# mattmireles/Mamba-ASR

Measured on AMD Instinct MI355X. Metric: encoder audio-frames/sec (ConMamba-large, L=4000), higher is better.
Workload: dtype bf16; 1 GPU; conmamba_large_ctc: encoder forward, 64 utterances x 4000 frames (1000 scan steps) per GPU, random-init weights; global_batch=64, frames_per_utterance=4000, parallelism=utterance shards x1 (no collective in forward), launch=hipGraph replay, streams=2 (join)

## Files before the change

### include/conmamba_hip.h

```cpp
#ifndef CONMAMBA_HIP_H
#define CONMAMBA_HIP_H

#include <stdint.h>

#ifdef __cplusplus
extern "C" {
#endif

#define CM_ABI_VERSION 12

#define CM_OK            0
#define CM_EINVAL       (-1)
#define CM_EUNSUPPORTED (-2)
#define CM_EALIGN       (-3)

typedef enum { CM_F32 = 0, CM_BF16 = 1, CM_F16 = 2 } cm_dtype;

#define CM_SCAN_CHUNK 64

int         cm_abi_version(void);
const char *cm_last_error(void);
int         cm_scan_num_chunks(int seqlen);
#ifdef CM_ABLATE
int         cm_debug_set(int ablation);
// ... 511 lines not shown
    const float *chan_mask;
    int32_t mask_rows, mask_c;
} cm_layernorm_args;

int64_t cm_layernorm_bwd_workspace_floats(int64_t rows, int32_t dim);
int cm_layernorm_fwd(const cm_layernorm_args *args);
int cm_layernorm_bwd(const cm_layernorm_args *args);

typedef struct cm_ln_pw_glu_args {
    int32_t rows, dim;
    const float *x;
    const void  *y;
    const float *ln_g, *ln_b;
    const void  *w;
    const float *bias;
    float *x_out;
    void  *out;
    float alpha, eps;
    void *stream;
} cm_ln_pw_glu_args;

int cm_ln_pw_glu(const cm_ln_pw_glu_args *args);

typedef struct cm_cnn_block1_args {
    int32_t batch, T, F, C;
    int32_t io_dtype;
    int32_t pad_out;
    const float *feats;
    const float *weight;
    const float *bias;
    const float *ln_g, *ln_b;
    float eps, slope;
    void *out;
    void *stream;
} cm_cnn_block1_args;

int cm_cnn_block1(const cm_cnn_block1_args *args);

typedef struct cm_cnn_block2_args {
    int32_t batch, T_in, F_in, C_in, C_out;
    int32_t pad_;
    const void  *in;
    const void  *weight;
    const float *bias;
    const float *ln_g, *ln_b;
    float eps, slope;
// ... 139 lines not shown
```

### mamba_asr_amd/_native.py

```python
from __future__ import annotations

import ctypes as C
import os

_HERE = os.path.dirname(os.path.abspath(__file__))
LIB_PATH = os.environ.get("CM_LIB_PATH") or os.path.join(_HERE, "lib", "libconmamba_hip.so")

CM_F32, CM_BF16, CM_F16 = 0, 1, 2
CM_SCAN_CHUNK = 64
CM_CTC_PREFIX_TILE_C, CM_CTC_PREFIX_TCHUNK = 64, 512
CM_BEAM_SELECT_MAX_B, CM_BEAM_SELECT_CHUNK = 128, 5120
CM_ATTN_STEP_MAX_T, CM_ATTN_STEP_MAX_H = 4096, 32
CM_XATTN_STEP_MAX_T, CM_XATTN_STEP_MAX_H = 8192, 32
ABI_VERSION = 12

i32, i64, vp, fp = C.c_int32, C.c_int64, C.c_void_p, C.c_void_p


class ScanFwdArgs(C.Structure):
    _fields_ = [
        ("batch", i32), ("dim", i32), ("seqlen", i32), ("dstate", i32),
        ("io_dtype", i32), ("bc_dtype", i32), ("delta_softplus", i32), ("reverse_time", i32),
        ("u", vp), ("delta", vp), ("A", fp), ("B", vp), ("C", vp), ("D", fp), ("z", vp), ("delta_bias", fp),
        ("out", vp), ("out_z", vp), ("x", fp),
# ... 157 lines not shown

class DwconvClArgs(C.Structure):
    _fields_ = [
        ("batch", i32), ("dim", i32), ("seqlen", i32), ("ksize", i32), ("pad_left", i32), ("io_dtype", i32),
        ("x", vp), ("weight", fp), ("bias", fp), ("y", vp), ("dy", vp), ("dx", vp), ("dweight", fp), ("dbias", fp), ("partial", fp),
        ("x_bs", i64), ("x_ts", i64), ("y_bs", i64), ("y_ts", i64), ("dy_bs", i64), ("dy_ts", i64), ("dx_bs", i64), ("dx_ts", i64),
        ("stream", vp), ("overwrite", i32), ("reserved0", i32),
    ]


class LayerNormArgs(C.Structure):
    _fields_ = [
        ("rows", i64), ("dim", i32), ("x_dtype", i32), ("y_dtype", i32), ("eps", C.c_float),
        ("x", vp), ("gamma", fp), ("beta", fp), ("y", vp), ("mean", fp), ("rstd", fp),
        ("dy", vp), ("dx", vp), ("dgamma", fp), ("dbeta", fp), ("workspace", fp), ("stream", vp), ("dres", fp),
        ("act", i32), ("act_slope", C.c_float), ("chan_mask", fp), ("mask_rows", i32), ("mask_c", i32),
    ]


class LnPwGluArgs(C.Structure):
    _fields_ = [
        ("rows", i32), ("dim", i32), ("x", fp), ("y", vp), ("ln_g", fp), ("ln_b", fp), ("w", vp), ("bias", fp),
        ("x_out", fp), ("out", vp), ("alpha", C.c_float), ("eps", C.c_float), ("stream", vp),
    ]


class CnnFrontArgs(C.Structure):
    _fields_ = [
        ("batch", i32), ("T", i32), ("F", i32), ("C1", i32), ("C2", i32), ("pad_", i32),
        ("feats", fp), ("w1", fp), ("b1", fp), ("ln1_g", fp), ("ln1_b", fp), ("w2", vp), ("b2", fp), ("ln2_g", fp), ("ln2_b", fp),
        ("eps1", C.c_float), ("eps2", C.c_float), ("slope", C.c_float), ("pad2_", i32), ("out", vp), ("stream", vp),
    ]


class AddLnArgs(C.Structure):
    _fields_ = [
        ("rows", i64), ("dim", i32), ("y_dtype", i32), ("out_dtype", i32), ("out_act", i32),
        ("x", fp), ("y", vp), ("alpha", C.c_float), ("eps1", C.c_float), ("eps2", C.c_float), ("pad2_", i32),
        ("g1", fp), ("b1", fp), ("g2", fp), ("b2", fp), ("x_out", fp), ("out", vp), ("stream", vp),
    ]


class GluDwconvArgs(C.Structure):
    _fields_ = [
        ("batch", i32), ("seqlen", i32), ("dim", i32), ("ksize", i32), ("io_dtype", i32), ("glu_done", i32),
        ("in_", vp), ("weight", fp), ("bias", fp), ("ln_g", fp), ("ln_b", fp), ("eps", C.c_float), ("variant", i32),
# ... 132 lines not shown
    ("cm_wgrad_bf16", C.c_int, [C.POINTER(WgradArgs)]),
    ("cm_scan_cl_bwd", C.c_int, [C.POINTER(ScanClBwdArgs)]),
    ("cm_conv_cl_fwd", C.c_int, [C.POINTER(ConvClArgs)]),
    ("cm_sum_leading", C.c_int, [vp, vp, i32, i64, i32, i32, vp]),
    ("cm_ctc_workspace_floats", C.c_int64, [i32, i32, i32]),
    ("cm_ctc_loss", C.c_int, [C.POINTER(CtcArgs)]),
    ("cm_ctc_beam_workspace_bytes", C.c_int64, [C.POINTER(CtcBeamArgs)]),
    ("cm_ctc_beam_search", C.c_int, [C.POINTER(CtcBeamArgs)]),
    ("cm_ctc_prefix_score", C.c_int, [C.POINTER(CtcPrefixArgs)]),
    ("cm_ctc_prefix_advance", C.c_int, [C.POINTER(CtcPrefixArgs)]),
    ("cm_beam_select_workspace_bytes", C.c_int64, [i32, i32, i32]),
    ("cm_beam_select", C.c_int, [C.POINTER(BeamSelectArgs)]),
    ("cm_attn_step", C.c_int, [C.POINTER(AttnStepArgs)]),
    ("cm_xattn_step", C.c_int, [C.POINTER(XattnStepArgs)]),
    ("cm_bias_act_dropout_bwd_workspace_floats", C.c_int64, [i64, i32]),
    ("cm_bias_act_dropout_fwd", C.c_int, [C.POINTER(FfnElemArgs)]),
    ("cm_bias_act_dropout_bwd", C.c_int, [C.POINTER(FfnElemArgs)]),
    ("cm_conv_cl_bwd_workspace_floats", C.c_int64, [i32, i32, i32]),
    ("cm_conv_cl_bwd", C.c_int, [C.POINTER(ConvClBwdArgs)]),
    ("cm_conv_xproj", C.c_int, [C.POINTER(ConvXprojArgs)]),
    ("cm_add_layernorm", C.c_int, [C.POINTER(AddLnArgs)]),
    ("cm_glu_dwconv_ln_gelu", C.c_int, [C.POINTER(GluDwconvArgs)]),
    ("cm_ln_pw_glu", C.c_int, [C.POINTER(LnPwGluArgs)]),
    ("cm_causal_conv1d_update", C.c_int, [C.POINTER(ConvUpdateArgs)]),
    ("cm_selective_state_update", C.c_int, [C.POINTER(StateUpdateArgs)]),
    ("cm_mamba_step", C.c_int, [C.POINTER(MambaStepArgs)]),
    ("cm_layernorm_bwd_workspace_floats", C.c_int64, [i64, i32]),
    ("cm_layernorm_fwd", C.c_int, [C.POINTER(LayerNormArgs)]),
    ("cm_layernorm_bwd", C.c_int, [C.POINTER(LayerNormArgs)]),
    ("cm_dwconv_cl_workspace_floats", C.c_int64, [i32, i32, i32]),
    ("cm_dwconv_cl_fwd", C.c_int, [C.POINTER(DwconvClArgs)]),
    ("cm_dwconv_cl_bwd", C.c_int, [C.POINTER(DwconvClArgs)]),
    ("cm_dwconv1d_fwd", C.c_int, [C.POINTER(Dwconv1dArgs)]),
    ("cm_dwconv1d_bwd", C.c_int, [C.POINTER(Dwconv1dArgs)]),
    ("cm_cnn_block1", C.c_int, [C.POINTER(CnnBlock1Args)]),
    ("cm_cnn_block2", C.c_int, [C.POINTER(CnnBlock2Args)]),
    ("cm_cnn_front", C.c_int, [C.POINTER(CnnFrontArgs)]),
    ("cm_gemm_bf16", C.c_int, [C.POINTER(GemmArgs)]),
    ("cm_ffn_fused", C.c_int, [C.POINTER(FfnArgs)]),
    ("cm_ffn_pack_weights", C.c_int, [vp, i32, i32, vp, vp]),
    ("cm_fbank_mel_db", C.c_int, [C.POINTER(FbankArgs)]),
    ("cm_fbank_finish", C.c_int, [C.POINTER(FbankArgs)]),
    ("cm_fbank_wav", C.c_int, [C.POINTER(FbankArgs)]),
    ("cm_spec_drop", C.c_int, [C.POINTER(SpecDropArgs)]),
]

# ... 31 lines not shown
```

### mamba_asr_amd/csrc/ln_pw_glu.hip

```cpp
#include "cm_common.h"


namespace {

typedef __attribute__((ext_vector_type(8))) __bf16 bf16x8;
typedef __attribute__((ext_vector_type(2))) __bf16 bf16x2;
typedef __attribute__((ext_vector_type(4))) float f32x4;
typedef __attribute__((ext_vector_type(2))) float f32x2;

constexpr int D = 256;
constexpr int TOK = 64;
constexpr int XS = 264;

__device__ __forceinline__ void lds_barrier() { asm volatile("s_waitcnt lgkmcnt(0)\n\ts_barrier" ::: "memory"); }
__device__ __forceinline__ uint32_t pack2(float a, float b) {
    return __builtin_bit_cast(uint32_t, __builtin_convertvector(f32x2{a, b}, bf16x2));
}

template <int OCC, int PF>
__global__ __launch_bounds__(256, OCC) void ln_pw_glu_kernel(const cm_ln_pw_glu_args p) {
    __shared__ __attribute__((aligned(16))) uint16_t xn[TOK * XS];
    const int tid = threadIdx.x, lane = tid & 63;
    const int wave = __builtin_amdgcn_readfirstlane(tid >> 6);
    const int l15 = lane & 15, lq = lane >> 4;
    const int t0 = blockIdx.x * TOK, M = p.rows;
    const uint16_t *yv = reinterpret_cast<const uint16_t *>(p.y);

    const __amdgpu_buffer_rsrc_t wr = __builtin_amdgcn_make_buffer_rsrc(const_cast<void *>(p.w), 0, 2 * D * D * 2, 0x00020000);
    const int vl = lane * 16;
    auto wload = [&](int ps, int s, bf16x8(&dst)[2]) {
        const int half = s >> 3, ks = s & 7;
#pragma unroll
        for (int mb = 0; mb < 2; ++mb)
            dst[mb] = __builtin_bit_cast(bf16x8, __builtin_amdgcn_raw_buffer_load_b128(
                                                     wr, vl, (((half * D + wave * 64) / 16 + 2 * ps + mb) * (D / 32) + ks) * 1024, 0));
    };
    bf16x8 wq[PF][2];
#pragma unroll
    for (int s = 0; s < PF; ++s) wload(0, s, wq[s]);

    {
        float4 v[4][4];
#pragma unroll
        for (int rd = 0; rd < 4; ++rd) {
            const int tok = min(t0 + wave * 16 + rd * 4 + lq, M - 1);
#pragma unroll
            for (int i = 0; i < 4; ++i) {
                const int col = (l15 + 16 * i) * 4;
                float4 x4 = *reinterpret_cast<const float4 *>(p.x + (int64_t)tok * D + col);
                if (yv) {
                    const uint2 a = *reinterpret_cast<const uint2 *>(yv + (int64_t)tok * D + col);
                    x4.x = fmaf(p.alpha, cm_bf16_lo(a.x), x4.x);
                    x4.y = fmaf(p.alpha, cm_bf16_hi(a.x), x4.y);
                    x4.z = fmaf(p.alpha, cm_bf16_lo(a.y), x4.z);
                    x4.w = fmaf(p.alpha, cm_bf16_hi(a.y), x4.w);
                }
                v[rd][i] = x4;
            }
        }
#pragma unroll
        for (int rd = 0; rd < 4; ++rd) {
            const int tok = t0 + wave * 16 + rd * 4 + lq;
            if (p.x_out && tok < M) {
#pragma unroll
                for (int i = 0; i < 4; ++i) *reinterpret_cast<float4 *>(p.x_out + (int64_t)tok * D + (l15 + 16 * i) * 4) = v[rd][i];
            }
            float s = 0.f;
#pragma unroll
            for (int i = 0; i < 4; ++i) s += (v[rd][i].x + v[rd][i].y) + (v[rd][i].z + v[rd][i].w);
            const float mean = cm_group_sum<16>(s) * (1.f / D);
            float q = 0.f;
#pragma unroll
            for (int i = 0; i < 4; ++i) {
                v[rd][i].x -= mean; v[rd][i].y -= mean; v[rd][i].z -= mean; v[rd][i].w -= mean;
                q = fmaf(v[rd][i].x, v[rd][i].x, fmaf(v[rd][i].y, v[rd][i].y, fmaf(v[rd][i].z, v[rd][i].z, fmaf(v[rd][i].w, v[rd][i].w, q))));
            }
            const float rstd = rsqrtf(cm_group_sum<16>(q) * (1.f / D) + p.eps);
            uint16_t *dst = xn + (wave * 16 + rd * 4 + lq) * XS;
#pragma unroll
            for (int i = 0; i < 4; ++i) {
                const int col = (l15 + 16 * i) * 4;
                const float4 g = *reinterpret_cast<const float4 *>(p.ln_g + col);
                const float4 b = *reinterpret_cast<const float4 *>(p.ln_b + col);
                uint2 pk;
                pk.x = pack2(fmaf(v[rd][i].x * rstd, g.x, b.x), fmaf(v[rd][i].y * rstd, g.y, b.y));
                pk.y = pack2(fmaf(v[rd][i].z * rstd, g.z, b.z), fmaf(v[rd][i].w * rstd, g.w, b.w));
                *reinterpret_cast<uint2 *>(dst + col) = pk;
            }
        }
    }
    lds_barrier();

    const uint16_t *xfrag = xn + l15 * XS + lq * 8;
    auto read_frags = [&](int ks, bf16x8(&bf)[4]) {
#pragma unroll
        for (int nb = 0; nb < 4; ++nb) bf[nb] = *reinterpret_cast<const bf16x8 *>(xfrag + nb * 16 * XS + ks * 32);
    };
    uint16_t *out = reinterpret_cast<uint16_t *>(p.out);
    uint2 held[2][4];
#pragma unroll
    for (int ps = 0; ps < 2; ++ps) {
        f32x4 acc[2][2][4];
#pragma unroll
        for (int h = 0; h < 2; ++h)
#pragma unroll
            for (int mb = 0; mb < 2; ++mb)
#pragma unroll
                for (int nb = 0; nb < 4; ++nb) acc[h][mb][nb] = f32x4{0.f, 0.f, 0.f, 0.f};
        bf16x8 bfa[4], bfb[4];
        read_frags(0, bfa);
#pragma unroll
        for (int s = 0; s < 16; ++s) {
// ... 32 lines not shown
    lds_barrier();
#pragma unroll
    for (int i = 0; i < TOK * 32 / 256; ++i) {
        const int idx = tid + 256 * i, row = idx >> 5, chunk = idx & 31;
        const uint4 v = *reinterpret_cast<const uint4 *>(xn + row * XS + chunk * 8);
        if (t0 + row < M) *reinterpret_cast<uint4 *>(out + (int64_t)(t0 + row) * D + chunk * 8) = v;
    }
}

}

extern "C" int cm_ln_pw_glu(const cm_ln_pw_glu_args *args) {
    CM_REQUIRE(args != nullptr, CM_EINVAL, "ln_pw_glu: args is NULL");
    const cm_ln_pw_glu_args &a = *args;
    CM_REQUIRE(a.rows > 0 && a.x && a.ln_g && a.ln_b && a.w && a.bias && a.out, CM_EINVAL, "ln_pw_glu: bad sizes or NULL tensor");
    CM_REQUIRE(a.dim == D, CM_EUNSUPPORTED, "ln_pw_glu: d_model must be 256 (got %d)", a.dim);
    CM_REQUIRE(cm_aligned(a.x, 16) && cm_aligned(a.ln_g, 16) && cm_aligned(a.ln_b, 16) && cm_aligned(a.w, 16) && cm_aligned(a.bias, 16) &&
                   cm_aligned(a.out, 16) && (!a.y || cm_aligned(a.y, 8)) && (!a.x_out || cm_aligned(a.x_out, 16)),
               CM_EALIGN, "ln_pw_glu: tensors must be 16-byte aligned (y / out 8)");
    const dim3 grid((a.rows + TOK - 1) / TOK);
    hipStream_t st = reinterpret_cast<hipStream_t>(a.stream);
#ifdef CM_ABLATE
    if (cm_debug_get() == 41) {
        hipLaunchKernelGGL((ln_pw_glu_kernel<3, 4>), grid, dim3(256), 0, st, a);
        return cm_launch_status("cm_ln_pw_glu");
    }
#endif
    hipLaunchKernelGGL((ln_pw_glu_kernel<4, 2>), grid, dim3(256), 0, st, a);
    return cm_launch_status("cm_ln_pw_glu");
}
```

### mamba_asr_amd/fused.py

```python
from __future__ import annotations

import os
from typing import Dict, Optional

import torch
import torch.nn.functional as F

from . import ops, weight_cache


class _LayerCache:

    def __init__(self, layer, dtype):
        self.dtype = dtype
        c = lambda t: t.detach().to(dtype).contiguous()
        f = lambda t: None if t is None else t.detach().float().contiguous()
        ffn = lambda m: dict(ln=(f(m[0].weight), f(m[0].bias), m[0].eps), w1=c(m[1].ffn[0].weight), b1=c(m[1].ffn[0].bias),
                             w2=c(m[1].ffn[3].weight), b2=c(m[1].ffn[3].bias), b1f=f(m[1].ffn[0].bias),
                             b2f=f(m[1].ffn[3].bias))
        self.ffn1, self.ffn2 = ffn(layer.ffn_module1), ffn(layer.ffn_module2)
        if ops.ffn_supported(self.ffn1["w1"].shape[1], self.ffn1["w1"].shape[0], dtype) and self.ffn1["w1"].is_cuda:
            for q in (self.ffn1, self.ffn2):
                q["w1p"], q["w2p"] = ops.PackedWeight(q["w1"], ops.FFN_LAYOUT), ops.PackedWeight(q["w2"], ops.FFN_LAYOUT)
                if ops.SMALL_FFN_ROWS > 0:
# ... 21 lines not shown
            self.dirs.append(dict(conv_w=f(conv.weight).reshape(m.d_inner, -1), conv_b=f(conv.bias), x_proj=c(xp.weight),
                                  dt_proj=c(dtp.weight), dt_proj_f32=c(dtp.weight).float().contiguous(), dt_bias=f(dtp.bias), A=(-torch.exp(A_log.detach().float())).contiguous(),
                                  D=f(getattr(m, "D_b" if sfx else "D"))))
        cm = layer.convolution_module
        self.x_proj_bd = torch.block_diag(m.x_proj.weight.detach().to(dtype), m.x_proj_b.weight.detach().to(dtype))
        R, N = self.dt_rank, self.d_state
        self.rows_mode = (R <= 16 or (R <= 32 and dtype == torch.bfloat16)) and N == 16 and m.d_inner % 8 == 0
        if self.rows_mode:
            pad = ops.rows_dt_pad(R)
            self.row_width = pad + 32
            rows = [ops.xproj_rows(xp.weight, R, pad, dtype) for xp in (m.x_proj, m.x_proj_b)]
            self.x_proj_rows = torch.block_diag(*rows)
            self.wx_packed = None
            if dtype == torch.bfloat16 and m.d_inner % 32 == 0 and m.d_inner <= 2048 and rows[0].is_cuda and m.d_conv == 4:
                self.wx_packed = [ops.PackedWeight(r) for r in rows]
            for d_, dtp in zip(self.dirs, (m.dt_proj, m.dt_proj_b)):
                d_["dt_w16"] = ops.pad_dt_weight(dtp.weight.detach().to(dtype))
        self.cm_ln = (f(cm.layer_norm.weight), f(cm.layer_norm.bias), cm.layer_norm.eps)
        self.pw_w, self.pw_b = c(cm.bottleneck[0].weight.squeeze(-1)), c(cm.bottleneck[0].bias)
        self.pw_bf, self.lin_bf = f(cm.bottleneck[0].bias), f(cm.after_conv[2].bias)
        self.pw_packed = None
        if dtype == torch.bfloat16 and self.pw_w.is_cuda and tuple(self.pw_w.shape) == (512, 256) and self.pw_bf is not None:
            self.pw_packed = ops.PackedWeight(self.pw_w)
        self.in_bias_f = None if m.in_proj.bias is None else f(m.in_proj.bias)
        self.out_bias_f = None if m.out_proj.bias is None else f(m.out_proj.bias)
        self.dw_w, self.dw_b = f(cm.conv.weight), f(cm.conv.bias)
        self.dw_wt = self.dw_w.reshape(self.dw_w.shape[0], -1).t().contiguous()
        self.cm_ln2 = (f(cm.after_conv[0].weight), f(cm.after_conv[0].bias), cm.after_conv[0].eps)
        self.lin_w, self.lin_b = c(cm.after_conv[2].weight), c(cm.after_conv[2].bias)
        self.lin_packed = None
        if USE_DWCONV_LIN and dtype == torch.bfloat16 and self.lin_w.is_cuda and tuple(self.lin_w.shape) == (256, 256) and self.lin_bf is not None:
            self.lin_packed = ops.PackedWeight(self.lin_w)
        self.kernel_size = cm.kernel_size


def _params_key(dtype, *modules):
    return (dtype,) + tuple((p._version, p.data_ptr()) for m in modules for p in m.parameters())


_LAYER = weight_cache.Kind("_cm_fused_cache", graphs_read=False, build=_LayerCache)


def _cache(layer, dtype) -> _LayerCache:
    return _LAYER.lookup(layer, _params_key(dtype, layer), dtype)


# ... 31 lines not shown
    if c.rows_mode and USE_SCAN_ROWS:
        if xdbl is None:
            xdbl = (ucat.view(rows, 2 * E) @ c.x_proj_rows.t()).view(batch, seqlen, 2 * c.row_width)
        RW = c.row_width
        return [dict(u=ucat[:, :, i * E:(i + 1) * E], A=d["A"], D=d["D"], delta_bias=d["dt_bias"], dt_weight=d["dt_w16"],
                     xdbl=xdbl[:, :, RW * i:RW * (i + 1)], out=ycat[:, :, i * E:(i + 1) * E], reverse=bool(i))
                for i, d in enumerate(c.dirs)]
    xdblT = c.x_proj_bd @ ucat.view(rows, 2 * E).t()
    feat = ops.alloc_bc(2 * P, batch, seqlen, ucat.device)
    feat.view(2 * P, rows).copy_(xdblT)
    dirs = []
    for i, d in enumerate(c.dirs):
        f = feat[i * P:(i + 1) * P]
        dd = dict(u=ucat[:, :, i * E:(i + 1) * E], A=d["A"], B=f[R:R + N], C=f[R + N:], D=d["D"],
                  delta_bias=d["dt_bias"], out=ycat[:, :, i * E:(i + 1) * E], reverse=bool(i))
        if R <= 16:
            dd.update(dt_low=f[:R], dt_weight=d["dt_proj_f32"])
        else:
            dd["delta"] = (xdblT[i * P:i * P + R].t() @ d["dt_proj"].t()).view(batch, seqlen, E)
        dirs.append(dd)
    return dirs


def bimamba_fused(c: _LayerCache, h, batch, seqlen, xz=None):
    E, R, N = c.d_inner, c.dt_rank, c.d_state
    rows = batch * seqlen
    if xz is None:
        xz = h @ c.in_proj.t()
        if c.in_bias is not None:
            xz = xz + c.in_bias
    xz3 = xz.view(batch, seqlen, 2 * E)
    ucat = torch.empty((batch, seqlen, 2 * E), dtype=xz.dtype, device=xz.device)
    xdbl = None
    if USE_CONV_XPROJ and USE_SCAN_ROWS and c.rows_mode and c.wx_packed is not None and xz.dtype == torch.bfloat16:
        xdbl = ops.conv_xproj(xz3[:, :, :E], c.dirs[0]["conv_w"], c.dirs[0]["conv_b"], c.dirs[1]["conv_w"], c.dirs[1]["conv_b"],
                              c.wx_packed[0], c.wx_packed[1], out_f=ucat[:, :, :E], out_b=ucat[:, :, E:])
    else:
        ops.conv_cl_fwd(xz3[:, :, :E], c.dirs[0]["conv_w"], c.dirs[0]["conv_b"], c.dirs[1]["conv_w"], c.dirs[1]["conv_b"],
                        True, out_f=ucat[:, :, :E], out_b=ucat[:, :, E:])
    ycat = torch.empty_like(ucat)
    dirs = _scan_dirs(c, ucat, ycat, batch, seqlen, xdbl)
    ops.scan_cl_fwd(dirs, z=xz3[:, :, E:], delta_softplus=True)
    y = ycat.view(rows, 2 * E) @ c.out_cat.t()
    if c.out_bias is not None:
        y = y + c.out_bias
    if c.gamma is not None:
        y = y * c.gamma.to(y.dtype)
    return y


USE_FUSED_FFN = os.environ.get("CM_FUSED_FFN", "1") == "1"


USE_LN_PW_GLU = os.environ.get("CM_LN_PW_GLU", "1") == "1"


def _layer_forward_ffn_fused(c, x, batch, seqlen, dtype, final_ln=None):
    D = x.shape[-1]
    f1, f2 = c.ffn1, c.ffn2
    if 0 < x.shape[0] <= ops.SMALL_FFN_ROWS and "w1s" in f1:
        f1 = dict(f1, w1p=f1["w1s"], w2p=f1["w2s"])
        f2 = dict(f2, w1p=f2["w1s"], w2p=f2["w2s"])
        inp = getattr(c, "in_packed_s", None)
    else:
        inp = c.in_packed
    if c.in_packed is not None:
        _, xz = ops.ffn_fused(x, f1["ln"], f1["w1p"], f1["b1f"], f1["w2p"], f1["b2f"], alpha=0.5, norm2=c.norm1, proj_w=inp)
        y = bimamba_fused(c, None, batch, seqlen, xz=xz)
    else:
        _, h = ops.ffn_fused(x, f1["ln"], f1["w1p"], f1["b1f"], f1["w2p"], f1["b2f"], alpha=0.5, norm2=c.norm1)
        y = bimamba_fused(c, h, batch, seqlen)
    if USE_LN_PW_GLU and c.pw_packed is not None and y.dtype == torch.bfloat16 and y.is_contiguous():
        gl = ops.ln_pw_glu(x, y, 1.0, c.cm_ln, c.pw_packed, c.pw_bf)
        g = ops.glu_dwconv_ln_gelu(gl.view(batch, seqlen, D), c.dw_w, c.dw_b, c.cm_ln2[0], c.cm_ln2[1], c.cm_ln2[2],
                                   weight_t=c.dw_wt, glu_done=True, lin_w=c.lin_packed, lin_b=c.lin_bf)
    else:
        _, h = ops.add_layernorm(x, y, 1.0, x_out=x, norm2=c.cm_ln, out_dtype=dtype)
        pw = torch.addmm(c.pw_b, h, c.pw_w.t()).view(batch, seqlen, 2 * D)
        g = ops.glu_dwconv_ln_gelu(pw, c.dw_w, c.dw_b, c.cm_ln2[0], c.cm_ln2[1], c.cm_ln2[2], weight_t=c.dw_wt,
                                   lin_w=c.lin_packed, lin_b=c.lin_bf)
    y = g if c.lin_packed is not None else torch.addmm(c.lin_b, g.view(-1, D), c.lin_w.t())
    if final_ln is not None:
        _, out = ops.ffn_fused(x, f2["ln"], f2["w1p"], f2["b1f"], f2["w2p"], f2["b2f"], alpha=0.5, addend=y.view(-1, D),
                               norm1=c.norm2, norm2=final_ln, h_dtype=torch.float32)
        return out, None
    ops.ffn_fused(x, f2["ln"], f2["w1p"], f2["b1f"], f2["w2p"], f2["b2f"], alpha=0.5, addend=y.view(-1, D), norm1=c.norm2,
                  want_h=False)
    return x, None


def layer_forward(layer, x, batch, seqlen, dtype, next_ln=None, final_ln=None):
    c = _cache(layer, dtype)
    D = x.shape[-1]
    if USE_FUSED_FFN and ops.ffn_supported(D, c.ffn1["w1"].shape[0], dtype) and c.ffn2["w1"].shape[0] == c.ffn1["w1"].shape[0]:
        return _layer_forward_ffn_fused(c, x, batch, seqlen, dtype, final_ln)
    _, h = ops.add_layernorm(x, None, norm2=c.ffn1["ln"], out_dtype=dtype)
# ... 102 lines not shown
                        ops.ffn_fused(xp, f1["ln"], f1["w1p"], f1["b1f"], f1["w2p"], f1["b2f"], alpha=0.5, norm2=c.norm1,
                                      proj_w=c.in_packed, proj_out=xz[b0:b1].view(-1, 2 * E))
                    else:
                        _, h = ops.ffn_fused(xp, f1["ln"], f1["w1p"], f1["b1f"], f1["w2p"], f1["b2f"], alpha=0.5, norm2=c.norm1)
                        torch.mm(h, c.in_proj.t(), out=xz[b0:b1].view(-1, 2 * E))
                    ops.conv_xproj(xz[b0:b1, :, :E], c.dirs[0]["conv_w"], c.dirs[0]["conv_b"], c.dirs[1]["conv_w"], c.dirs[1]["conv_b"],
                                   c.wx_packed[0], c.wx_packed[1], out_f=ucat[b0:b1, :, :E], out_b=ucat[b0:b1, :, E:], xdbl=xdbl[b0:b1])
            if paired:
                for pi, (b0, b1) in enumerate(parts):
                    with torch.cuda.stream(streams[pi]):
                        if gate is not None:
                            streams[pi].wait_event(gate)
                        ops.scan_cl_fwd(_scan_dirs(c, ucat[b0:b1], ycat[b0:b1], b1 - b0, seqlen, xdbl[b0:b1]), z=xz[b0:b1, :, E:],
                                        delta_softplus=True)
                        gate = torch.cuda.Event()
                        gate.record(streams[pi])
            else:
                join()
                ops.scan_cl_fwd(_scan_dirs(c, ucat, ycat, batch, seqlen, xdbl), z=xz[:, :, E:], delta_softplus=True)
                fork()
            for pi, (b0, b1) in enumerate(parts):
                with torch.cuda.stream(streams[pi]):
                    xp = x[b0 * seqlen:b1 * seqlen]
                    y = ycat[b0:b1].view(-1, 2 * E) @ c.out_cat.t()
                    gl = ops.ln_pw_glu(xp, y, 1.0, c.cm_ln, c.pw_packed, c.pw_bf)
                    g = ops.glu_dwconv_ln_gelu(gl.view(b1 - b0, seqlen, D), c.dw_w, c.dw_b, c.cm_ln2[0], c.cm_ln2[1], c.cm_ln2[2],
                                               weight_t=c.dw_wt, glu_done=True, lin_w=c.lin_packed, lin_b=c.lin_bf)
                    yl = g.view(-1, D) if c.lin_packed is not None else torch.addmm(c.lin_b, g.view(-1, D), c.lin_w.t())
                    if li == n - 1:
                        _, outs[pi] = ops.ffn_fused(xp, f2["ln"], f2["w1p"], f2["b1f"], f2["w2p"], f2["b2f"], alpha=0.5, addend=yl,
                                                    norm1=c.norm2, norm2=fin, h_dtype=torch.float32)
                    else:
                        ops.ffn_fused(xp, f2["ln"], f2["w1p"], f2["b1f"], f2["w2p"], f2["b2f"], alpha=0.5, addend=yl, norm1=c.norm2,
                                      want_h=False)
        join()
        for o in outs[1:]:
            o.record_stream(cur)
        return torch.cat(outs, dim=0).view(batch, seqlen, D)


@torch.no_grad()
def encoder_forward(encoder, src, dtype: Optional[torch.dtype] = None, streams: Optional[int] = None):
    if dtype is None:
        dtype = torch.get_autocast_dtype("cuda") if torch.is_autocast_enabled("cuda") else torch.float32
    ns = min(N_STREAMS, max(1, src.shape[0] // 16)) if streams is None else streams
    if ns > 1 and src.shape[0] >= 2 * 8 and STREAM_MODE in ("join", "pair"):
        out = _encoder_forward_joined(encoder, src, dtype, ns, paired=STREAM_MODE == "pair")
        if out is not None:
# ... 116 lines not shown
```

### mamba_asr_amd/ops.py

```python
from __future__ import annotations

import ctypes as ct
from typing import Optional, Tuple

import math
import os

import torch

from . import _native as N
from . import weight_cache
from .weight_cache import invalidate_caches

_DT = {torch.float32: N.CM_F32, torch.bfloat16: N.CM_BF16, torch.float16: N.CM_F16}


DETERMINISTIC = os.environ.get("CM_DETERMINISTIC", "1") == "1"


LAUNCH_LOG: Optional[list] = None


def _launch(name: str, fn, args, units: int = 0):
    log = LAUNCH_LOG
# ... 1315 lines not shown
class LnActDropFn(torch.autograd.Function):

    @staticmethod
    def forward(ctx, x, weight, bias, eps, slope, chan_mask, out_dtype):
        b, t, f, c = x.shape
        x2 = x.reshape(b * t, f * c)
        y, x2s, stats = layernorm_fwd(x2, weight, bias, eps, out_dtype, leaky_slope=slope, chan_mask=chan_mask, mask_rows=t)
        ctx.save_for_backward(x2s, stats, weight, bias, chan_mask if chan_mask is not None else weight.new_empty(0))
        ctx.cfg = (eps, slope, t, chan_mask is not None, x.shape)
        return y.view(x.shape)

    @staticmethod
    def backward(ctx, dy):
        x2, stats, weight, bias, mask = ctx.saved_tensors
        eps, slope, t, has_mask, shape = ctx.cfg
        if dy.dtype not in (torch.float32, torch.bfloat16):
            dy = dy.float()
        dy = dy if dy.is_contiguous() else dy.contiguous()
        dx, dg, db = layernorm_bwd(dy.view(x2.shape[0], -1), x2, stats, weight, eps, need_dx=ctx.needs_input_grad[0], bias=bias, leaky_slope=slope,
                                   chan_mask=mask if has_mask else None, mask_rows=t)
        return (dx.view(shape) if dx is not None else None), dg.to(weight.dtype), db.to(weight.dtype), None, None, None, None


def ln_pw_glu(x, y, alpha, norm, w, bias, x_out=None):
    _dev_check(x, y, bias)
    rows, d = x.shape
    if x.dtype != torch.float32 or not x.is_contiguous() or d != 256:
        raise RuntimeError("ln_pw_glu: x must be a contiguous fp32 (rows, 256) tensor")
    if y is not None and (y.dtype != torch.bfloat16 or not y.is_contiguous() or y.shape != x.shape):
        raise RuntimeError("ln_pw_glu: y must be a contiguous bf16 (rows, 256) tensor")
    if not isinstance(w, PackedWeight) or w.shape != (512, 256):
        raise RuntimeError("ln_pw_glu: w must be a PackedWeight of shape (512, 256)")
    g_, b_, bs = _f32c(norm[0]), _f32c(norm[1]), _f32c(bias)
    xo = x if x_out is None else x_out
    out = torch.empty((rows, d), dtype=torch.bfloat16, device=x.device)
    a = N.LnPwGluArgs()
    a.rows, a.dim, a.x, a.y, a.ln_g, a.ln_b, a.w, a.bias = rows, d, _ptr(x), _ptr(y), _ptr(g_), _ptr(b_), _ptr(w.data), _ptr(bs)
    a.x_out, a.out, a.alpha, a.eps, a.stream = _ptr(xo), _ptr(out), float(alpha), float(norm[2]), _stream()
    _launch("cm_ln_pw_glu", N.lib().cm_ln_pw_glu, a, units=rows)
    return out


def glu_dwconv_ln_gelu(inp, weight, bias, ln_weight, ln_bias, eps=1e-5, weight_t=None, glu_done=False, lin_w=None, lin_b=None,
                       variant: int = 0):
    _dev_check(inp, weight, bias, ln_weight, ln_bias)
    if not inp.is_contiguous():
        inp = inp.contiguous()
    b, l, d2 = inp.shape
    d = d2 if glu_done else d2 // 2
    w = _f32c(weight).reshape(d, -1)
    bs, g, bt = _f32c(bias), _f32c(ln_weight), _f32c(ln_bias)
    out = torch.empty((b, l, d), dtype=inp.dtype, device=inp.device)
    a = N.GluDwconvArgs()
    a.batch, a.seqlen, a.dim, a.ksize, a.io_dtype, a.glu_done = b, l, d, w.shape[1], _DT[inp.dtype], int(bool(glu_done))
    a.in_, a.weight, a.bias, a.ln_g, a.ln_b, a.eps, a.out = _ptr(inp), _ptr(w), _ptr(bs), _ptr(g), _ptr(bt), float(eps), _ptr(out)
    wt = w.t().contiguous() if weight_t is None else weight_t
    if wt.dtype != torch.float32 or wt.shape != (w.shape[1], d) or not wt.is_contiguous():
        raise RuntimeError("glu_dwconv_ln_gelu: weight_t must be a contiguous fp32 (k, dim) tensor")
# ... 326 lines not shown
```

### mamba_asr_amd/seqpar.py

```python
from __future__ import annotations

from typing import List, Optional, Sequence, Tuple

import torch
import torch.distributed as dist
import torch.nn.functional as F


class DistGroup:

    def __init__(self, group=None):
        self.group = group
        self.rank, self.world = dist.get_rank(group), dist.get_world_size(group)

    def all_gather(self, t: torch.Tensor) -> List[torch.Tensor]:
        out = [torch.empty_like(t) for _ in range(self.world)]
        dist.all_gather(out, t.contiguous(), group=self.group)
        return out


class _ThreadRank:
    def __init__(self, shared, rank, world):
        self._s, self.rank, self.world = shared, rank, world

# ... 174 lines not shown
            xz = (h @ c.in_proj.t()).view(batch, T, 2 * E)
            left, right = exchange_halo(xz[:, :, :E], 3, 3, group, dim=1)
            xext = torch.cat([left, xz[:, :, :E], right], dim=1)
            uext = torch.empty((batch, T + 6, 2 * E), dtype=dtype, device=dev)
            xdbl_ext = ops.conv_xproj(xext, c.dirs[0]["conv_w"], c.dirs[0]["conv_b"], c.dirs[1]["conv_w"], c.dirs[1]["conv_b"],
                                      c.wx_packed[0], c.wx_packed[1], out_f=uext[:, :, :E], out_b=uext[:, :, E:])
            ucat, xdbl = uext[:, 3:3 + T], xdbl_ext[:, 3:3 + T]
            ycat = torch.empty((batch, T, 2 * E), dtype=dtype, device=dev)
            summ = torch.empty((2, 2, batch, E, 16), dtype=torch.float32, device=dev)
            dirs = [dict(u=ucat[:, :, i * E:(i + 1) * E], A=d["A"], D=d["D"], delta_bias=d["dt_bias"], dt_weight=d["dt_w16"],
                         xdbl=xdbl[:, :, 48 * i:48 * (i + 1)], out=ycat[:, :, i * E:(i + 1) * E], reverse=bool(i),
                         decay=summ[i, 0], h_last=summ[i, 1]) for i, d in enumerate(c.dirs)]
            ops.scan_cl_fwd(dirs, z=xz[:, :, E:], delta_softplus=True)
            allsum = group.all_gather(summ)
            redo = []
            for i in range(2):
                H = carry_in([s_[i, 0] for s_ in allsum], [s_[i, 1] for s_ in allsum], group.rank, bool(i))
                if H is not None:
                    dd = {k: v for k, v in dirs[i].items() if k not in ("decay", "h_last")}
                    dd["h0"] = H.contiguous()
                    redo.append(dd)
            if redo:
                ops.scan_cl_fwd(redo, z=xz[:, :, E:], delta_softplus=True)
            y = ycat.view(batch * T, 2 * E) @ c.out_cat.t()
            gl = ops.ln_pw_glu(x, y, 1.0, c.cm_ln, c.pw_packed, c.pw_bf)
            gl3 = gl.view(batch, T, D)
            left, right = exchange_halo(gl3, 15, 15, group, dim=1)
            g = ops.glu_dwconv_ln_gelu(torch.cat([left, gl3, right], dim=1), c.dw_w, c.dw_b, c.cm_ln2[0], c.cm_ln2[1], c.cm_ln2[2],
                                       weight_t=c.dw_wt, glu_done=True)[:, 15:15 + T]
            yl = torch.addmm(c.lin_b, g.reshape(-1, D), c.lin_w.t())
            if li == len(caches) - 1:
                _, out = ops.ffn_fused(x, f2["ln"], f2["w1p"], f2["b1f"], f2["w2p"], f2["b2f"], alpha=0.5, addend=yl, norm1=c.norm2,
                                       norm2=fin, h_dtype=torch.float32)
            else:
                ops.ffn_fused(x, f2["ln"], f2["w1p"], f2["b1f"], f2["w2p"], f2["b2f"], alpha=0.5, addend=yl, norm1=c.norm2, want_h=False)
        return out.view(batch, T, D)


def exchange_bytes_per_layer(batch: int, d_model: int, expand: int = 2, d_state: int = 16, d_conv: int = 4, kernel_size: int = 31,
                             itemsize: int = 4) -> int:
    E = expand * d_model
    scan = 2 * 2 * batch * E * d_state * 4
    halos = 2 * batch * E * (d_conv - 1) * itemsize + batch * d_model * (kernel_size - 1) * itemsize
    return scan + halos
```

Baseline: 20.67 million audio-frames/s.

## Fuse Mamba out-projection GEMM into the LayerNorm/pointwise-GLU kernel

Adds a MIX variant of the ln_pw_glu kernel that computes the bidirectional-Mamba out-projection (ycat @ out_cat^T) in-kernel. The ycat tiles are streamed into LDS with double-buffered buffer_load...lds DMA, and the projection weights are prefetched into registers. The bf16 result lands in the shared token tile and feeds the residual-add/LayerNorm/pointwise-GLU path, so the separate hipBLAS GEMM and its (rows,256) bf16 intermediate round-trip to HBM go away. The trade-off is more per-block work and register pressure in a kernel that keeps occupancy 4, and the GEMM now runs with a 64-token tile and only 256 threads per block.

```diff
diff --git a/include/conmamba_hip.h b/include/conmamba_hip.h
--- a/include/conmamba_hip.h
+++ b/include/conmamba_hip.h
@@ -557,6 +557,23 @@
 
 int cm_ln_pw_glu(const cm_ln_pw_glu_args *args);
 
+typedef struct cm_ln_pw_glu_mix_args {
+    int32_t rows, dim;
+    const float *x;
+    const float *ln_g, *ln_b;
+    const void  *w;
+    const float *bias;
+    float *x_out;
+    void  *out;
+    float alpha, eps;
+    void *stream;
+    const void *ycat;
+    const void *proj_w;
+    int32_t proj_k;
+} cm_ln_pw_glu_mix_args;
+
+int cm_ln_pw_glu_mix(const cm_ln_pw_glu_mix_args *args);
+
 typedef struct cm_cnn_block1_args {
     int32_t batch, T, F, C;
     int32_t io_dtype;
diff --git a/mamba_asr_amd/_native.py b/mamba_asr_amd/_native.py
--- a/mamba_asr_amd/_native.py
+++ b/mamba_asr_amd/_native.py
@@ -203,6 +203,14 @@
     _fields_ = [
         ("rows", i32), ("dim", i32), ("x", fp), ("y", vp), ("ln_g", fp), ("ln_b", fp), ("w", vp), ("bias", fp),
         ("x_out", fp), ("out", vp), ("alpha", C.c_float), ("eps", C.c_float), ("stream", vp),
+    ]
+
+
+class LnPwGluMixArgs(C.Structure):
+    _fields_ = [
+        ("rows", i32), ("dim", i32), ("x", fp), ("ln_g", fp), ("ln_b", fp), ("w", vp), ("bias", fp),
+        ("x_out", fp), ("out", vp), ("alpha", C.c_float), ("eps", C.c_float), ("stream", vp),
+        ("ycat", vp), ("proj_w", vp), ("proj_k", i32),
     ]
 
 
@@ -381,6 +389,7 @@
     ("cm_add_layernorm", C.c_int, [C.POINTER(AddLnArgs)]),
     ("cm_glu_dwconv_ln_gelu", C.c_int, [C.POINTER(GluDwconvArgs)]),
     ("cm_ln_pw_glu", C.c_int, [C.POINTER(LnPwGluArgs)]),
+    ("cm_ln_pw_glu_mix", C.c_int, [C.POINTER(LnPwGluMixArgs)]),
     ("cm_causal_conv1d_update", C.c_int, [C.POINTER(ConvUpdateArgs)]),
     ("cm_selective_state_update", C.c_int, [C.POINTER(StateUpdateArgs)]),
     ("cm_mamba_step", C.c_int, [C.POINTER(MambaStepArgs)]),
diff --git a/mamba_asr_amd/csrc/ln_pw_glu.hip b/mamba_asr_amd/csrc/ln_pw_glu.hip
--- a/mamba_asr_amd/csrc/ln_pw_glu.hip
+++ b/mamba_asr_amd/csrc/ln_pw_glu.hip
@@ -7,6 +7,7 @@
 typedef __attribute__((ext_vector_type(2))) __bf16 bf16x2;
 typedef __attribute__((ext_vector_type(4))) float f32x4;
 typedef __attribute__((ext_vector_type(2))) float f32x2;
+typedef __attribute__((ext_vector_type(4))) unsigned int u32x4;
 
 constexpr int D = 256;
 constexpr int TOK = 64;
@@ -17,8 +18,30 @@
     return __builtin_bit_cast(uint32_t, __builtin_convertvector(f32x2{a, b}, bf16x2));
 }
 
-template <int OCC, int PF>
-__global__ __launch_bounds__(256, OCC) void ln_pw_glu_kernel(const cm_ln_pw_glu_args p) {
+constexpr int CK = 128;
+constexpr int STAGE = TOK * CK * 2;
+static_assert(2 * STAGE <= TOK * XS * 2, "the two ycat stages must fit the token tile they overlay");
+
+struct mix_extra {
+    const void *ycat;
+    const void *proj_w;
+    int32_t proj_k;
+};
+
+__device__ __forceinline__ u32x4 raw_rsrc(const void *base, uint32_t bytes) {
+    const uint64_t a = reinterpret_cast<uint64_t>(base);
+    return u32x4{(uint32_t)a, (uint32_t)(a >> 32) & 0xffffu, bytes, 0x00020000u};
+}
+__device__ __forceinline__ void dma16(const u32x4 rsrc, uint32_t lds_addr, int voff) {
+    uint32_t keep;
+    asm volatile("s_mov_b32 %0, m0\n\ts_mov_b32 m0, %1\n\ts_nop 0\n\tbuffer_load_dwordx4 %2, %3, 0 offen lds\n\ts_mov_b32 m0, %0"
+                 : "=&s"(keep)
+                 : "s"(lds_addr), "v"(voff), "s"(rsrc)
+                 : "memory");
+}
+
+template <int OCC, int PF, bool MIX>
+__global__ __launch_bounds__(256, OCC) void ln_pw_glu_kernel(const cm_ln_pw_glu_args p, const mix_extra mx) {
     __shared__ __attribute__((aligned(16))) uint16_t xn[TOK * XS];
     const int tid = threadIdx.x, lane = tid & 63;
     const int wave = __builtin_amdgcn_readfirstlane(tid >> 6);
@@ -36,8 +59,77 @@
                                                      wr, vl, (((half * D + wave * 64) / 16 + 2 * ps + mb) * (D / 32) + ks) * 1024, 0));
     };
     bf16x8 wq[PF][2];
-#pragma unroll
-    for (int s = 0; s < PF; ++s) wload(0, s, wq[s]);
+    if constexpr (MIX) {
+        static_assert(PF == 2, "the projection phase's ring indexing assumes two steps in flight");
+        const int K = mx.proj_k, kt = K / 32, nch = K / CK, nstep = 2 * kt;
+        const __amdgpu_buffer_rsrc_t pr = __builtin_amdgcn_make_buffer_rsrc(const_cast<void *>(mx.proj_w), 0, D * K * 2, 0x00020000);
+        auto pload = [&](int g, bf16x8(&dst)[2]) {
+            g = min(g, nstep - 1);
+            const int ks = g >> 1, mp = g & 1;
+#pragma unroll
+            for (int mb = 0; mb < 2; ++mb)
+                dst[mb] = __builtin_bit_cast(bf16x8, __builtin_amdgcn_raw_buffer_load_b128(pr, vl, ((wave * 4 + mp * 2 + mb) * kt + ks) * 1024, 0));
+        };
+        const int vrows = min(TOK, M - t0);
+        const u32x4 yr = raw_rsrc(reinterpret_cast<const unsigned char *>(mx.ycat) + (int64_t)t0 * K * 2, (uint32_t)(vrows * K * 2));
+        const uint32_t lds0 = (uint32_t)reinterpret_cast<uintptr_t>(&xn[0]);
+        int go[4];
+#pragma unroll
+        for (int i = 0; i < 4; ++i) {
+            const int row = 4 * (4 * wave + i) + lq;
+            go[i] = row * K * 2 + 16 * (l15 ^ (((row & 3) << 2) | ((row >> 2) & 3)));
+        }
+        auto request = [&](int c) {
+#pragma unroll
+            for (int i = 0; i < 4; ++i) dma16(yr, lds0 + (uint32_t)((c & 1) * STAGE + (4 * wave + i) * 1024), go[i] + c * (CK * 2));
+        };
+        request(0);
+#pragma unroll
+        for (int s = 0; s < PF; ++s) pload(s, wq[s]);
+        f32x4 acc[4][4];
+#pragma unroll
+        for (int mb = 0; mb < 4; ++mb)
+#pragma unroll
+            for (int nb = 0; nb < 4; ++nb) acc[mb][nb] = f32x4{0.f, 0.f, 0.f, 0.f};
+        const unsigned char *xb = reinterpret_cast<const unsigned char *>(xn);
+        const int yrow = l15 * (CK * 2), yswz = ((l15 & 3) << 2) | (l15 >> 2);
+        auto read_y = [&](int st, int kk, bf16x8(&bf)[4]) {
+            const int off = st * STAGE + yrow + 16 * ((kk * 4 + lq) ^ yswz);
+#pragma unroll
+            for (int nb = 0; nb < 4; ++nb) bf[nb] = *reinterpret_cast<const bf16x8 *>(xb + off + nb * 16 * (CK * 2));
+        };
+        for (int c = 0; c < nch; ++c) {
+            asm volatile("s_waitcnt vmcnt(0)" ::: "memory");
+            lds_barrier();
+            if (c + 1 < nch) request(c + 1);
+            const int st = c & 1;
+            bf16x8 bf[4];
+#pragma unroll
+            for (int s = 0; s < 8; ++s) {
+                const int kk = s >> 1, mp = s & 1;
+                if (mp == 0) read_y(st, kk, bf);
+#pragma unroll
+                for (int mb = 0; mb < 2; ++mb)
+#pragma unroll
+                    for (int nb = 0; nb < 4; ++nb)
+                        acc[mp * 2 + mb][nb] = __builtin_amdgcn_mfma_f32_16x16x32_bf16(wq[s % PF][mb], bf[nb], acc[mp * 2 + mb][nb], 0, 0, 0);
+                pload(c * 8 + s + PF, wq[s % PF]);
+                __builtin_amdgcn_sched_barrier(0);
+            }
+        }
+        lds_barrier();
+#pragma unroll
+        for (int mb = 0; mb < 4; ++mb)
+#pragma unroll
+            for (int nb = 0; nb < 4; ++nb)
+                *reinterpret_cast<uint2 *>(xn + (nb * 16 + l15) * XS + wave * 64 + mb * 16 + lq * 4) =
+                    uint2{pack2(acc[mb][nb][0], acc[mb][nb][1]), pack2(acc[mb][nb][2], acc[mb][nb][3])};
+    }
+    if constexpr (MIX) lds_barrier();
+    else {
+#pragma unroll
+        for (int s = 0; s < PF; ++s) wload(0, s, wq[s]);
+    }
 
     {
         float4 v[4][4];
@@ -48,8 +140,9 @@
             for (int i = 0; i < 4; ++i) {
                 const int col = (l15 + 16 * i) * 4;
                 float4 x4 = *reinterpret_cast<const float4 *>(p.x + (int64_t)tok * D + col);
-                if (yv) {
-                    const uint2 a = *reinterpret_cast<const uint2 *>(yv + (int64_t)tok * D + col);
+                if (MIX || yv) {
+                    const uint2 a = MIX ? *reinterpret_cast<const uint2 *>(xn + (wave * 16 + rd * 4 + lq) * XS + col)
+                                        : *reinterpret_cast<const uint2 *>(yv + (int64_t)tok * D + col);
                     x4.x = fmaf(p.alpha, cm_bf16_lo(a.x), x4.x);
                     x4.y = fmaf(p.alpha, cm_bf16_hi(a.x), x4.y);
                     x4.z = fmaf(p.alpha, cm_bf16_lo(a.y), x4.z);
@@ -88,6 +181,10 @@
                 *reinterpret_cast<uint2 *>(dst + col) = pk;
             }
         }
+    }
+    if constexpr (MIX) {
+#pragma unroll
+        for (int s = 0; s < PF; ++s) wload(0, s, wq[s]);
     }
     lds_barrier();
 
@@ -166,10 +263,37 @@
     hipStream_t st = reinterpret_cast<hipStream_t>(a.stream);
 #ifdef CM_ABLATE
     if (cm_debug_get() == 41) {
-        hipLaunchKernelGGL((ln_pw_glu_kernel<3, 4>), grid, dim3(256), 0, st, a);
+        hipLaunchKernelGGL((ln_pw_glu_kernel<3, 4, false>), grid, dim3(256), 0, st, a, mix_extra{});
         return cm_launch_status("cm_ln_pw_glu");
     }
 #endif
-    hipLaunchKernelGGL((ln_pw_glu_kernel<4, 2>), grid, dim3(256), 0, st, a);
+    hipLaunchKernelGGL((ln_pw_glu_kernel<4, 2, false>), grid, dim3(256), 0, st, a, mix_extra{});
     return cm_launch_status("cm_ln_pw_glu");
 }
+
+extern "C" int cm_ln_pw_glu_mix(const cm_ln_pw_glu_mix_args *args) {
+    CM_REQUIRE(args != nullptr, CM_EINVAL, "ln_pw_glu_mix: args is NULL");
+    const cm_ln_pw_glu_mix_args &m = *args;
+    CM_REQUIRE(m.rows > 0 && m.x && m.ln_g && m.ln_b && m.w && m.bias && m.out && m.ycat && m.proj_w, CM_EINVAL,
+               "ln_pw_glu_mix: bad sizes or NULL tensor");
+    CM_REQUIRE(m.dim == D, CM_EUNSUPPORTED, "ln_pw_glu_mix: d_model must be 256 (got %d)", m.dim);
+    CM_REQUIRE(m.proj_k >= CK && m.proj_k % CK == 0 && m.proj_k <= 8192, CM_EUNSUPPORTED,
+               "ln_pw_glu_mix: proj_k must be a multiple of 128, at most 8192 (got %d)", m.proj_k);
+    CM_REQUIRE(cm_aligned(m.x, 16) && cm_aligned(m.ln_g, 16) && cm_aligned(m.ln_b, 16) && cm_aligned(m.w, 16) && cm_aligned(m.bias, 16) &&
+                   cm_aligned(m.out, 16) && cm_aligned(m.ycat, 16) && cm_aligned(m.proj_w, 16) && (!m.x_out || cm_aligned(m.x_out, 16)),
+               CM_EALIGN, "ln_pw_glu_mix: tensors must be 16-byte aligned");
+    const auto overlap = [](const void *a, int64_t na, const void *b, int64_t nb) {
+        const uintptr_t pa = reinterpret_cast<uintptr_t>(a), pb = reinterpret_cast<uintptr_t>(b);
+        return a && b && pa < pb + (uintptr_t)nb && pb < pa + (uintptr_t)na;
+    };
+    const int64_t nx = (int64_t)m.rows * D * 4, no = (int64_t)m.rows * D * 2, ny = (int64_t)m.rows * m.proj_k * 2;
+    CM_REQUIRE(!overlap(m.out, no, m.x, nx) && !overlap(m.out, no, m.ycat, ny) && !overlap(m.out, no, m.x_out, nx) &&
+                   !overlap(m.x_out, nx, m.ycat, ny) && (m.x_out == m.x || !overlap(m.x_out, nx, m.x, nx)),
+               CM_EALIGN, "ln_pw_glu_mix: out / x_out overlap an input (only x_out == x is allowed)");
+    cm_ln_pw_glu_args a{};
+    a.rows = m.rows, a.dim = m.dim, a.x = m.x, a.y = nullptr, a.ln_g = m.ln_g, a.ln_b = m.ln_b, a.w = m.w, a.bias = m.bias;
+    a.x_out = m.x_out, a.out = m.out, a.alpha = m.alpha, a.eps = m.eps, a.stream = m.stream;
+    const mix_extra mx{m.ycat, m.proj_w, m.proj_k};
+    hipLaunchKernelGGL((ln_pw_glu_kernel<4, 2, true>), dim3((a.rows + TOK - 1) / TOK), dim3(256), 0, reinterpret_cast<hipStream_t>(a.stream), a, mx);
+    return cm_launch_status("cm_ln_pw_glu_mix");
+}
diff --git a/mamba_asr_amd/fused.py b/mamba_asr_amd/fused.py
--- a/mamba_asr_amd/fused.py
+++ b/mamba_asr_amd/fused.py
@@ -67,6 +67,10 @@
         self.pw_packed = None
         if dtype == torch.bfloat16 and self.pw_w.is_cuda and tuple(self.pw_w.shape) == (512, 256) and self.pw_bf is not None:
             self.pw_packed = ops.PackedWeight(self.pw_w)
+        self.out_packed = None
+        if (self.pw_packed is not None and self.out_cat.is_cuda and self.out_cat.shape[0] == 256 and self.out_cat.shape[1] % 128 == 0
+                and self.out_cat.shape[1] <= 8192 and self.out_bias is None and self.gamma is None):
+            self.out_packed = ops.PackedWeight(self.out_cat)
         self.in_bias_f = None if m.in_proj.bias is None else f(m.in_proj.bias)
         self.out_bias_f = None if m.out_proj.bias is None else f(m.out_proj.bias)
         self.dw_w, self.dw_b = f(cm.conv.weight), f(cm.conv.bias)
@@ -144,7 +148,25 @@
     return dirs
 
 
-def bimamba_fused(c: _LayerCache, h, batch, seqlen, xz=None):
+USE_MIXER_TAIL = os.environ.get("CM_MIXER_TAIL", "1") == "1"
+
+
+def _out_proj(c: _LayerCache, ycat):
+    y = ycat @ c.out_cat.t()
+    if c.out_bias is not None:
+        y = y + c.out_bias
+    if c.gamma is not None:
+        y = y * c.gamma.to(y.dtype)
+    return y
+
+
+def mixer_tail(c: _LayerCache, x, ycat):
+    if USE_MIXER_TAIL and c.out_packed is not None:
+        return ops.ln_pw_glu(x, None, 1.0, c.cm_ln, c.pw_packed, c.pw_bf, ycat=ycat, out_w=c.out_packed)
+    return ops.ln_pw_glu(x, _out_proj(c, ycat), 1.0, c.cm_ln, c.pw_packed, c.pw_bf)
+
+
+def bimamba_fused(c: _LayerCache, h, batch, seqlen, xz=None, want_ycat=False):
     E, R, N = c.d_inner, c.dt_rank, c.d_state
     rows = batch * seqlen
     if xz is None:
@@ -163,12 +185,9 @@
     ycat = torch.empty_like(ucat)
     dirs = _scan_dirs(c, ucat, ycat, batch, seqlen, xdbl)
     ops.scan_cl_fwd(dirs, z=xz3[:, :, E:], delta_softplus=True)
-    y = ycat.view(rows, 2 * E) @ c.out_cat.t()
-    if c.out_bias is not None:
-        y = y + c.out_bias
-    if c.gamma is not None:
-        y = y * c.gamma.to(y.dtype)
-    return y
+    if want_ycat:
+        return ycat.view(rows, 2 * E)
+    return _out_proj(c, ycat.view(rows, 2 * E))
 
 
 USE_FUSED_FFN = os.environ.get("CM_FUSED_FFN", "1") == "1"
@@ -186,14 +205,15 @@
         inp = getattr(c, "in_packed_s", None)
     else:
         inp = c.in_packed
+    seam = USE_LN_PW_GLU and c.pw_packed is not None and dtype == torch.bfloat16
     if c.in_packed is not None:
         _, xz = ops.ffn_fused(x, f1["ln"], f1["w1p"], f1["b1f"], f1["w2p"], f1["b2f"], alpha=0.5, norm2=c.norm1, proj_w=inp)
-        y = bimamba_fused(c, None, batch, seqlen, xz=xz)
+        y = bimamba_fused(c, None, batch, seqlen, xz=xz, want_ycat=seam)
     else:
         _, h = ops.ffn_fused(x, f1["ln"], f1["w1p"], f1["b1f"], f1["w2p"], f1["b2f"], alpha=0.5, norm2=c.norm1)
-        y = bimamba_fused(c, h, batch, seqlen)
-    if USE_LN_PW_GLU and c.pw_packed is not None and y.dtype == torch.bfloat16 and y.is_contiguous():
-        gl = ops.ln_pw_glu(x, y, 1.0, c.cm_ln, c.pw_packed, c.pw_bf)
+        y = bimamba_fused(c, h, batch, seqlen, want_ycat=seam)
+    if seam:
+        gl = mixer_tail(c, x, y)
         g = ops.glu_dwconv_ln_gelu(gl.view(batch, seqlen, D), c.dw_w, c.dw_b, c.cm_ln2[0], c.cm_ln2[1], c.cm_ln2[2],
                                    weight_t=c.dw_wt, glu_done=True, lin_w=c.lin_packed, lin_b=c.lin_bf)
     else:
@@ -342,8 +362,7 @@
             for pi, (b0, b1) in enumerate(parts):
                 with torch.cuda.stream(streams[pi]):
                     xp = x[b0 * seqlen:b1 * seqlen]
-                    y = ycat[b0:b1].view(-1, 2 * E) @ c.out_cat.t()
-                    gl = ops.ln_pw_glu(xp, y, 1.0, c.cm_ln, c.pw_packed, c.pw_bf)
+                    gl = mixer_tail(c, xp, ycat[b0:b1].view(-1, 2 * E))
                     g = ops.glu_dwconv_ln_gelu(gl.view(b1 - b0, seqlen, D), c.dw_w, c.dw_b, c.cm_ln2[0], c.cm_ln2[1], c.cm_ln2[2],
                                                weight_t=c.dw_wt, glu_done=True, lin_w=c.lin_packed, lin_b=c.lin_bf)
                     yl = g.view(-1, D) if c.lin_packed is not None else torch.addmm(c.lin_b, g.view(-1, D), c.lin_w.t())
diff --git a/mamba_asr_amd/ops.py b/mamba_asr_amd/ops.py
--- a/mamba_asr_amd/ops.py
+++ b/mamba_asr_amd/ops.py
@@ -1361,8 +1361,8 @@
         return (dx.view(shape) if dx is not None else None), dg.to(weight.dtype), db.to(weight.dtype), None, None, None, None
 
 
-def ln_pw_glu(x, y, alpha, norm, w, bias, x_out=None):
-    _dev_check(x, y, bias)
+def ln_pw_glu(x, y, alpha, norm, w, bias, x_out=None, ycat=None, out_w=None):
+    _dev_check(x, y, bias, ycat)
     rows, d = x.shape
     if x.dtype != torch.float32 or not x.is_contiguous() or d != 256:
         raise RuntimeError("ln_pw_glu: x must be a contiguous fp32 (rows, 256) tensor")
@@ -1373,6 +1373,19 @@
     g_, b_, bs = _f32c(norm[0]), _f32c(norm[1]), _f32c(bias)
     xo = x if x_out is None else x_out
     out = torch.empty((rows, d), dtype=torch.bfloat16, device=x.device)
+    if (ycat is None) != (out_w is None) or (ycat is not None and y is not None):
+        raise RuntimeError("ln_pw_glu: give either y, or ycat together with out_w")
+    if ycat is not None:
+        if ycat.dtype != torch.bfloat16 or not ycat.is_contiguous() or ycat.dim() != 2 or ycat.shape[0] != rows:
+            raise RuntimeError("ln_pw_glu: ycat must be a contiguous bf16 (rows, K) tensor")
+        if not isinstance(out_w, PackedWeight) or out_w.layout != 16 or out_w.shape != (256, ycat.shape[1]):
+            raise RuntimeError("ln_pw_glu: out_w must be a PackedWeight (16-row tiles) of shape (256, K)")
+        m = N.LnPwGluMixArgs()
+        m.rows, m.dim, m.x, m.ln_g, m.ln_b, m.w, m.bias = rows, d, _ptr(x), _ptr(g_), _ptr(b_), _ptr(w.data), _ptr(bs)
+        m.x_out, m.out, m.alpha, m.eps, m.stream = _ptr(xo), _ptr(out), float(alpha), float(norm[2]), _stream()
+        m.ycat, m.proj_w, m.proj_k = _ptr(ycat), _ptr(out_w.data), ycat.shape[1]
+        _launch("cm_ln_pw_glu", N.lib().cm_ln_pw_glu_mix, m, units=rows)
+        return out
     a = N.LnPwGluArgs()
     a.rows, a.dim, a.x, a.y, a.ln_g, a.ln_b, a.w, a.bias = rows, d, _ptr(x), _ptr(y), _ptr(g_), _ptr(b_), _ptr(w.data), _ptr(bs)
     a.x_out, a.out, a.alpha, a.eps, a.stream = _ptr(xo), _ptr(out), float(alpha), float(norm[2]), _stream()
diff --git a/mamba_asr_amd/seqpar.py b/mamba_asr_amd/seqpar.py
--- a/mamba_asr_amd/seqpar.py
+++ b/mamba_asr_amd/seqpar.py
@@ -220,8 +220,7 @@
                     redo.append(dd)
             if redo:
                 ops.scan_cl_fwd(redo, z=xz[:, :, E:], delta_softplus=True)
-            y = ycat.view(batch * T, 2 * E) @ c.out_cat.t()
-            gl = ops.ln_pw_glu(x, y, 1.0, c.cm_ln, c.pw_packed, c.pw_bf)
+            gl = fused.mixer_tail(c, x, ycat.view(batch * T, 2 * E))
             gl3 = gl.view(batch, T, D)
             left, right = exchange_halo(gl3, 15, 15, group, dim=1)
             g = ops.glu_dwconv_ln_gelu(torch.cat([left, gl3, right], dim=1), c.dw_w, c.dw_b, c.cm_ln2[0], c.cm_ln2[1], c.cm_ln2[2],
```

New measurement: 21.80 million audio-frames/s (median of 6 runs). 1.05x the previous value.
